# X1X1010/XequiNet

Measured on AMD Instinct MI355X. Metric: edges/sec + achieved HBM GB/s, energy+force inference, QM9-shape batch, higher is better.
Workload: dtype f32

## Files before the change

include/xeq.h:

```cpp
#ifndef XEQ_H
#define XEQ_H
#include <stdint.h>

#ifdef __cplusplus
extern "C" {
#endif

enum { XEQ_F32 = 0, XEQ_F64 = 1 };
enum { XEQ_RBF_BESSEL = 0, XEQ_RBF_GAUSSIAN = 1, XEQ_RBF_EXPBERN = 2, XEQ_RBF_EXPNORM = 3 };
enum { XEQ_CUTOFF_COSINE = 0, XEQ_CUTOFF_POLYNOMIAL = 1 };
enum {
  XEQ_OK = 0,
  XEQ_ERR_INVALID_ARGUMENT = 1,
  XEQ_ERR_LAUNCH = 2,
  XEQ_ERR_UNSUPPORTED = 3
};

int xeq_version(void);
const char* xeq_last_error(void);
int64_t xeq_launch_count(void);
int64_t xeq_launch_names(int64_t first, char* buf, int64_t cap);


int xeq_csr_rowptr(const int64_t* keys, int64_t n_keys, int64_t n_rows, int32_t* rowptr, void* stream);
// ... 236 lines not shown
int xeq_message_wq_supported(int num_basis, int node_dim, const int32_t mul[3]);
int xeq_message_wq_fits(int64_t n_nodes, int64_t n_edges, int num_basis, int node_dim, const int32_t mul[3]);
int64_t xeq_message_wq_pcap(int64_t n_nodes, int64_t n_edges);
int xeq_message_wq_waves(void);
int xeq_message_wq_record_floats_for(int num_basis);
int xeq_message_wq_record_floats(void);
int64_t xeq_message_wq_plan_workspace(int64_t n_nodes);
int64_t xeq_message_wq_win_ints(int n_ranges);
int xeq_message_wq_plan(const int32_t* rowptr, const int32_t* perm, const int64_t* owner, const int64_t* gather,
                        int64_t n_nodes, int64_t n_edges, int n_ranges, void* workspace, int64_t workspace_bytes,
                        int32_t* qptr, int32_t* pgath, int32_t* peid, int32_t* qinfo, int32_t* sq, int32_t* sn, int32_t* win,
                        void* stream);
int xeq_edge_basis_wq(const void* vec, int64_t n_nodes, int64_t n_edges, const int32_t* qptr, const int32_t* peid,
                      int rbf_kind, int cutoff_kind, int num_basis, double cutoff, const void* p0, const void* p1,
                      void* basis, void* dbasis, void* stream);
int xeq_message_fwd_wq(int64_t n_nodes, int64_t n_edges, int n_ranges, const int32_t* sq, const int32_t* sn, const int32_t* win,
                       const int32_t* c_rowptr, const int32_t* pgath, const int32_t* qinfo, const void* basis, const void* h,
                       const void* xhat, const void* s_in, const void* x_in, const void* w_rbf, const void* b_rbf,
                       int num_basis, int node_dim, const int32_t mul[3], void* s_out, void* x_out, int xhat_layout,
                       void* stream);
int64_t xeq_message_wq_parts_floats(int64_t n_nodes, int64_t n_edges, const int32_t mul[3]);
#define XEQ_XHAT_HIGHER_L_ZERO 2
#define XEQ_WQ_MIRROR_WALK 4
#define XEQ_WQ_PACKED_WEIGHTS 64
int64_t xeq_message_wq_packed_weight_floats(int num_basis, int node_dim, const int32_t mul[3]);
int xeq_message_wq_pack_weights(const void* w_rbf, const void* b_rbf, int num_basis, int node_dim, const int32_t mul[3], void* packed,
                                void* stream);
int xeq_message_bwd_wq(int64_t n_nodes, int64_t n_edges, int n_ranges, const int32_t* sq, const int32_t* sn, const int32_t* win,
                       const int32_t* n_rowptr, const int32_t* pgath, const int32_t* qinfo, const void* basis,
                       const void* dbasis, const void* h, const void* xhat, const void* grad_s, const void* grad_x,
                       const void* w_rbf, const void* b_rbf, int num_basis, int node_dim, const int32_t mul[3], void* grad_h,
                       void* grad_xhat, void* parts, int xhat_layout, void* stream);
int xeq_message_wq_table_max_rows(void);
int xeq_message_wq_first_table(int family, int64_t table_rows, int training, int per_node_front);
int xeq_edge_basis_wq_table(const void* vec, int64_t n_nodes, int64_t n_edges, const int32_t* qptr, const int32_t* peid,
                            int rbf_kind, int cutoff_kind, int num_basis, double cutoff, const void* p0, const void* p1,
                            void* basis, void* dbasis, const int32_t* pgath, const int32_t* qinfo, const void* z, int z_is_int64,
                            int64_t table_rows, int32_t* slot_rows, int32_t* quad_rows, void* stream);
int xeq_message_fwd_wq_table(int64_t n_nodes, int64_t n_edges, int n_ranges, const int32_t* sq, const int32_t* sn, const int32_t* win,
                             const int32_t* c_rowptr, const int32_t* slot_rows, const int32_t* qinfo, const void* basis,
                             const void* h_table, const void* xhat0_table, int64_t table_rows, const void* s_in, const void* x_in,
                             const void* w_rbf, const void* b_rbf, int num_basis, int node_dim, const int32_t mul[3], void* s_out,
                             void* x_out, int xhat_layout, void* stream);
int xeq_message_bwd_wq_table(int64_t n_nodes, int64_t n_edges, int n_ranges, const int32_t* sq, const int32_t* sn, const int32_t* win,
                             const int32_t* n_rowptr, const int32_t* pgath, const int32_t* qinfo, const int32_t* quad_rows,
                             const void* basis, const void* dbasis, const void* h_table, const void* xhat0_table, int64_t table_rows,
                             const void* grad_s, const void* grad_x, const void* w_rbf, const void* b_rbf, int num_basis, int node_dim,
                             const int32_t mul[3], void* parts, int xhat_layout, void* stream);
int xeq_message_wq_edge_grad(const void* vec, int64_t n_nodes, int64_t n_edges, const int32_t* qptr, const int32_t* peid,
                             const int32_t* mirror, const int32_t mul[3], const void* parts, void* grad_vec, void* stream);
#define XEQ_WQ_MAX_PART_SETS 8
int xeq_message_wq_edge_grad_sum(const void* vec, int64_t n_nodes, int64_t n_edges, const int32_t* qptr, const int32_t* peid,
                                 const int32_t* mirror, const int32_t mul[3], int n_sets, const void* const* parts, void* grad_vec,
                                 void* stream);


int xeq_norm_fwd(int dtype, const void* s, const void* x, const void* ln_w, const void* ln_b, const void* eq_w,
                 const void* eq_b, int64_t n, int node_dim, const int32_t mul[3], int do_norm, void* shat, int64_t ld_s,
                 void* xhat_bt, void* stats, void* stream);
int xeq_norm_bwd(int dtype, const void* s, const void* x, const void* ln_w, const void* eq_w, const void* stats,
                 int64_t n, int node_dim, const int32_t mul[3], int do_norm, const void* g_shat, int64_t ld_gs,
                 const void* g_xhat_bt, const void* res_s, const void* res_x, void* g_s, void* g_x, void* stream);
int xeq_uv_reduce_fwd(int dtype, const void* uv_bt, int64_t n, const int32_t mul[3], double eps, void* cat,
                      int64_t ld_cat, int node_dim, void* p, void* stream);
int xeq_uv_reduce_bwd(int dtype, const void* uv_bt, const void* g_p, const void* g_cat, int64_t ld_cat, int node_dim,
                      int64_t n, const int32_t mul[3], double eps, const void* g_x_out, const void* a, void* g_uv_bt,
// ... 145 lines not shown
```

xequinet_amd/csrc/xeq_message_wq.hip:

```cpp
#include "xeq_common.h"

#include <hipcub/hipcub.hpp>
#include <stdlib.h>

namespace xeq {

typedef float f32x16 __attribute__((ext_vector_type(16)));
typedef float f32x4 __attribute__((ext_vector_type(4)));
typedef int i32x4 __attribute__((ext_vector_type(4)));

typedef __bf16 bf16x8 __attribute__((ext_vector_type(8)));

constexpr bool wq_bftail(int ks) { return ks <= 3; }
constexpr int WQ_TAIL = 24;
constexpr int wq_tailw(int ks) { return ks <= 4 ? 4 : 8; }
constexpr int wq_recf(int ks) { return WQ_TAIL + 2 * wq_tailw(ks) + 8; }
constexpr int wq_yoff(int ks) { return WQ_TAIL + 2 * wq_tailw(ks); }
constexpr int wq_tail_values(int num_basis) { return (num_basis > 16 ? num_basis - 16 : 0) + 1; }
constexpr int wq_ks(int num_basis) {
  return wq_tail_values(num_basis) <= 1 ? 1 : (wq_tail_values(num_basis) <= 5 ? 3 : ((wq_tail_values(num_basis) + 1) / 2 < 4 ? 4 : (wq_tail_values(num_basis) + 1) / 2));
}
static_assert(wq_tailw(5) == wq_tailw(8) && wq_tailw(6) == wq_tailw(8) && wq_tailw(7) == wq_tailw(8) && !wq_bftail(5) && !wq_bftail(8),
              "records written for 5, 6 or 7 tail steps are read by the KS = 8 kernels");
constexpr int WQ_REC_MAX = 48;
// ... 343 lines not shown
  return 1;
}

__device__ __forceinline__ void wq_decode(const WqArgs& a, int nunits, int& s0, int& s1, int& unit) {
  const int b = blockIdx.x;
  int region, j;
  if (a.regions == 8) {
    region = b & 7;
    j = b >> 3;
  } else {
    region = 0;
    j = b;
  }
  const int c = j / nunits;
  unit = nunits - 1 - (j - c * nunits);
  const int base = region * a.region_steps, rend = min(base + a.region_steps, a.n_steps);
  s0 = s1 = 0;
  int cc = c;
#pragma unroll
  for (int v = 0; v < 3; ++v) {
    if (cc >= 0 && cc < a.lvl_chunks[v]) {
      const int lend = v < 2 ? base + a.lvl_start[v + 1] : rend;
      s0 = base + a.lvl_start[v] + cc * a.lvl_spw[v];
      s1 = min(s0 + a.lvl_spw[v], min(lend, rend));
    }
    cc -= a.lvl_chunks[v];
  }
}

#ifndef XEQ_WQ_WIN_FLOATS
#define XEQ_WQ_WIN_FLOATS 12288
#endif
constexpr int WQ_WIN_FLOATS = XEQ_WQ_WIN_FLOATS;
constexpr int WQ_TAB_MAX_ROWS = WQ_WIN_FLOATS * 4 / 512 < 128 ? WQ_WIN_FLOATS * 4 / 512 : 128;

template <int KS>
constexpr int WQ_WK = 3 * 64 * 4 + (wq_bftail(KS) ? 3 * 64 * 4 : KS * 64);
template <int KS>
__device__ __forceinline__ void wq_stage_weights(const WqArgs& a, const WqUnit& un, const float* __restrict__ w,
                                                 const float* __restrict__ b, float* wl) {
  const int nkind = un.l == 0 ? 3 : 2, B = a.B;
  if (a.packed_w) {
    const int unit_index = (un.l == 0 ? 0 : (un.l == 1 ? a.nu[0] : a.nu[0] + a.nu[1])) + un.cb;
    const f32x4* __restrict__ src = reinterpret_cast<const f32x4*>(w + (size_t)unit_index * (3 * WQ_WK<KS>));
    for (int idx = threadIdx.x; idx < nkind * WQ_WK<KS> / 4; idx += blockDim.x) reinterpret_cast<f32x4*>(wl)[idx] = src[idx];
    return;
  }
  auto row_of = [&](int kind, int ln) { return (kind == 0 ? un.u0 : (kind == 1 ? a.C + un.u0 : 2 * a.C + 32 * un.cb)) + (ln & 31); };
  for (int idx = threadIdx.x; idx < nkind * 3 * 64; idx += blockDim.x) {
    const int kind = idx / 192, rem = idx - 192 * kind, split = rem >> 6, ln = rem & 63;
    const int row = row_of(kind, ln), kh = ln >> 5;
    uint32_t pk[4] = {0u, 0u, 0u, 0u};
#pragma unroll
    for (int jj = 0; jj < 8; ++jj) {
      const int k = 8 * kh + jj;
      uint32_t a3[3];
      wq_split3(k < B ? w[(int64_t)row * B + k] : 0.f, a3[0], a3[1], a3[2]);
      pk[jj >> 1] |= a3[split] << (16 * (jj & 1));
    }
    *reinterpret_cast<f32x4*>(wl + kind * WQ_WK<KS> + 4 * (64 * split + ln)) =
        f32x4{__uint_as_float(pk[0]), __uint_as_float(pk[1]), __uint_as_float(pk[2]), __uint_as_float(pk[3])};
  }
  if constexpr (wq_bftail(KS)) {
    for (int idx = threadIdx.x; idx < nkind * 3 * 64; idx += blockDim.x) {
      const int kind = idx / 192, rem = idx - 192 * kind, v = rem >> 6, ln = rem & 63;
      const int row = row_of(kind, ln), kh = ln >> 5;
      uint32_t pk[4] = {0u, 0u, 0u, 0u};
#pragma unroll
      for (int jj = 0; jj < 8; ++jj) {
        const int slot = 8 * kh + jj, part = slot / 5, q = slot - 5 * part;
// ... 195 lines not shown
static __device__ unsigned long long g_wq_stamps[32];
static __device__ unsigned long long g_wq_wg[8192 * 4];
#ifdef XEQ_WQ_STAMPS
#define WQ_STAMP(i)                                                                                          \
  do {                                                                                                       \
    __builtin_amdgcn_sched_barrier(0);                                                                       \
    unsigned long long now_;                                                                                 \
    asm volatile("s_memtime %0\n\ts_waitcnt lgkmcnt(0)" : "=s"(now_)::"memory");                            \
    __builtin_amdgcn_sched_barrier(0);                                                                       \
    st_[i] += now_ - last_;                                                                                  \
    last_ = now_;                                                                                            \
  } while (0)
#else
#define WQ_STAMP(i) \
  do {              \
  } while (0)
#endif

__device__ __forceinline__ float wq_lds(const float* win, uint32_t byte_off) {
  return *reinterpret_cast<const float*>(reinterpret_cast<const char*>(win) + byte_off);
}
#ifndef XEQ_WQ_FWD_WPE
#define XEQ_WQ_FWD_WPE 2
#endif
#ifndef XEQ_WQ_BWD_WPE
#define XEQ_WQ_BWD_WPE 2
#endif

#ifndef XEQ_WQ_PART_BWD

template <int NM, bool XZ>
__device__ __forceinline__ void wq_stage_fwd(const WqArgs& a, const WqUnit& un, const WqCols& wc, const float* __restrict__ h,
                                             const float* __restrict__ xhat_, int w0, int nrows, float* win) {
  constexpr int NH = NM == 1 ? 3 : 2, NSL = NH + NM;
  if constexpr (XZ && NM > 1) {
    const int total = nrows * 8;
    for (int idx = threadIdx.x; idx < total; idx += blockDim.x) {
      const int row = idx >> 3, chunk = idx & 7;
      *reinterpret_cast<f32x4*>(win + (row * NSL + 1) * 32 + 4 * chunk) =
          *reinterpret_cast<const f32x4*>(h + (int64_t)(w0 + row) * a.H + a.C + un.u0 + 4 * chunk);
    }
    return;
  }
  const int total = nrows * NSL * 8;
  const int64_t xnode = wc.xnode_b / 4, xcomp = a.xl == 0 ? 32 : wc.xcomp_b / 4;
  constexpr int UN = 8;
  const int nthr = blockDim.x;
  for (int base = threadIdx.x; base < total; base += UN * nthr) {
    f32x4 v[UN];
#pragma unroll
    for (int k = 0; k < UN; ++k) {
      const int idx = base + k * nthr;
      const int piece = idx >> 3, chunk = idx & 7;
      const int row = piece / NSL, sl = piece - row * NSL;
      const int64_t n = w0 + (idx < total ? row : 0);
      const float* src = sl < NH ? h + n * a.H + (sl == 0 ? un.u0 : (sl == 1 ? a.C + un.u0 : 2 * a.C + 32 * un.cb))
                                 : xhat_ + wc.x_base + n * xnode + (sl - NH) * xcomp;
      v[k] = *reinterpret_cast<const f32x4*>(src + 4 * chunk);
    }
#pragma unroll
    for (int k = 0; k < UN; ++k) {
      const int idx = base + k * nthr;
      if (idx < total) *reinterpret_cast<f32x4*>(win + (idx >> 3) * 32 + 4 * (idx & 7)) = v[k];
    }
  }
}

constexpr int wq_tab_row_bytes(int NM) { return NM == 1 ? 512 : 128; }
template <int NM>
__device__ __forceinline__ void wq_stage_table_fwd(const WqArgs& a, const WqUnit& un, const float* __restrict__ h_tab,
                                                   const float* __restrict__ x0_tab, float* win) {
  constexpr int NP = NM == 1 ? 4 : 1;
  const int total = a.tab_rows * NP * 8;
  for (int idx = threadIdx.x; idx < total; idx += blockDim.x) {
    const int piece = idx >> 3, chunk = idx & 7;
    const int row = piece / NP, sl = piece - row * NP;
    const float* src = NM > 1 ? h_tab + (int64_t)row * a.H + a.C + un.u0
                              : (sl < 3 ? h_tab + (int64_t)row * a.H + (sl == 0 ? un.u0 : (sl == 1 ? a.C + un.u0 : 2 * a.C + 32 * un.cb))
                                        : x0_tab + (int64_t)row * a.F + un.u0);
    *reinterpret_cast<f32x4*>(win + piece * 32 + 4 * chunk) = *reinterpret_cast<const f32x4*>(src + 4 * chunk);
  }
}

template <int NM, int KS, bool WIN, bool XZ, bool FENCED, bool TAB = false>
__device__ __forceinline__ void wq_fwd_body(const WqArgs& a, int range, const WqUnit un, const WqCols& wc,
                                            const float* __restrict__ rec, const float* __restrict__ h,
                                            const float* __restrict__ xhat_, const float* __restrict__ s_in,
                                            const float* __restrict__ x_in, const float* wl, float* __restrict__ s_out,
                                            float* __restrict__ x_out, int* tbl, const float* win, int w0,
                                            unsigned long long* st_, unsigned long long& last_) {
  constexpr bool HAS_S = NM == 1;
  constexpr bool NO_STATE = XZ && NM > 1;
  constexpr int YOFF = NM == 3 ? 0 : 3;
  static_assert(!TAB || (WIN && (XZ || NM == 1)), "the table form is a window form of the first block");
  constexpr int NH = NM == 1 ? 3 : 2, ROWB = TAB ? wq_tab_row_bytes(NM) : (NH + NM) * 128;
  constexpr uint32_t HE_OFF = TAB && NM > 1 ? 0u : 128u;
  const int lane = threadIdx.x & 63, j = lane & 31, hh = lane >> 5;
  const uint32_t row_s = 4u * (uint32_t)a.F, row_x = 4u * (uint32_t)a.D;
  wq_for_isolated(a, range, lane, [&](int m) {
    if (hh == 0) {
      if constexpr (HAS_S) wq_st(s_out, (uint32_t)m * row_s + wc.b_s, wq_ld(s_in, (uint32_t)m * row_s + wc.b_s));
#pragma unroll
      for (int mm = 0; mm < NM; ++mm)
        wq_st(x_out, (uint32_t)m * row_x + wc.b_xe + 4u * mm, wq_ld(x_in, (uint32_t)m * row_x + wc.b_xe + 4u * mm));
    }
  });
  const WqStreams st = wq_streams(a, range, un.l == 0 ? a.mlong : 1);
  if (st.ntiles == 0) return;
  const float* __restrict__ h_e = h + a.C;
  const float* __restrict__ h_m = h + (2 * a.C + 32 * un.cb - un.u0);
  const float* xhat_m[NM];
#pragma unroll
  for (int m = 0; m < NM; ++m) xhat_m[m] = xhat_ + wc.x_base + (int64_t)m * (wc.xcomp_b / 4);
  const uint32_t stride0 = WIN ? (uint32_t)ROWB : 4u * (uint32_t)a.H, stride1 = WIN ? 0u : wc.xnode_b;
  const uint32_t gbase = WIN ? (uint32_t)w0 : 0u;
  uint32_t lxm[NM];
#pragma unroll
  for (int m = 0; m < NM; ++m) lxm[m] = (uint32_t)(NH * 128) + (a.xl == 0 ? 4u * (uint32_t)(j * NM + m) : (uint32_t)(128 * m + 4 * j));
  const float* Ws = wl;
  const float* We = wl + WQ_WK<KS>;
  const float* Wm = wl + 2 * WQ_WK<KS>;

  float acc_s = 0.f, acc_x[NM];
#pragma unroll
  for (int m = 0; m < NM; ++m) acc_x[m] = 0.f;

  using Row = WqRow<KS, 1, (NM > 1)>;
  Row row;
  wq_row<KS, 1, (NM > 1)>(a, st, lane, 0, rec, nullptr, row, (int)gbase);
  wq_publish<KS, 1, (NM > 1)>(lane, row, stride0, stride1, tbl, gbase);
  __builtin_amdgcn_wave_barrier();

#ifdef XEQ_WQ_DEFER_STORES
  constexpr bool DEFER_ST = NM <= 3;
#else
  constexpr bool DEFER_ST = false;
#endif
  float pend_x[DEFER_ST ? 4 : 1][NM], pend_s[DEFER_ST ? 4 : 1];
  uint32_t pend_ob[DEFER_ST ? 4 : 1], pend_os[DEFER_ST ? 4 : 1];
  int pend_last[DEFER_ST ? 4 : 1];
  if constexpr (DEFER_ST) {
#pragma unroll
    for (int g = 0; g < 4; ++g) pend_last[g] = 0;
  }
  auto flush_nodes = [&]() {
    if constexpr (DEFER_ST) {
#pragma unroll
      for (int g = 0; g < 4; ++g)
        if (pend_last[g]) {
#pragma unroll
          for (int m = 0; m < NM; ++m) wq_st(x_out, pend_ob[g] + 4u * m, pend_x[g][m]);
// ... 14 lines not shown
#pragma unroll
    for (int g = 0; g < 4; ++g) {
      uint32_t t0[4];
      wq_tread4<uint32_t>(tb, T_G0 + 16 * hh + 4 * g, t0);
#pragma unroll
      for (int r = 0; r < 4; ++r) g0[4 * g + r] = t0[r];
      if constexpr (!WIN) {
        uint32_t t1[4];
        wq_tread4<uint32_t>(tb, T_G1 + 16 * hh + 4 * g, t1);
#pragma unroll
        for (int r = 0; r < 4; ++r) g1[4 * g + r] = t1[r];
      }
      const uint32_t own = (uint32_t)tb[T_QOWN + 4 * hh + g];
      keep[g] = tb[T_QKEEP + 4 * hh + g];
      last[g] = tb[T_QLAST + 4 * hh + g];
      ob[g] = own * row_x + wc.b_xe;
      os[g] = own * row_s + wc.b_s;
#pragma unroll
      for (int m = 0; m < NM; ++m) res_x[g][m] = wq_ld(x_in, ob[g] + 4u * m);
      res_s[g] = HAS_S ? wq_ld(s_in, os[g]) : 0.f;
    }
    XEQ_WQ_FSB();
    wq_row<KS, 1, (NM > 1)>(a, st, lane, t + 1, rec, nullptr, row, (int)gbase);
    XEQ_WQ_FSB();
    WQ_STAMP(5);
#ifdef XEQ_WQ_FWD_GR
    constexpr int GR = NM == 5 && XEQ_WQ_FWD_GR > 4 ? XEQ_WQ_FWD_GR / 2 : XEQ_WQ_FWD_GR;
#else
    constexpr int GR = NM == 5 ? 8 : 16;
#endif
    f32x16 ds, de, dm;
#pragma unroll
    for (int r0 = 0; r0 < 16; r0 += GR) {
      float hs[GR], he[GR], hm[HAS_S ? GR : 1], xv[GR][NM];
#pragma unroll
      for (int u = 0; u < GR; ++u) {
        const int v = r0 + u;
        if constexpr (WIN) {
          const uint32_t oh = g0[v] + 4u * (uint32_t)j;
          if constexpr (!NO_STATE) hs[u] = wq_lds(win, oh);
          he[u] = wq_lds(win, oh + HE_OFF);
          if constexpr (HAS_S) hm[u] = wq_lds(win, oh + 256u);
          if constexpr (!NO_STATE) {
#pragma unroll
            for (int m = 0; m < NM; ++m) xv[u][m] = wq_lds(win, g0[v] + lxm[m]);
          }
        } else {
          const uint32_t oh = g0[v] + wc.b_hs, ox = g1[v] + wc.b_x;
          if constexpr (!NO_STATE) hs[u] = wq_ld(h, oh);
          he[u] = wq_ld(h_e, oh);
          if constexpr (HAS_S) hm[u] = wq_ld(h_m, oh);
          if constexpr (!NO_STATE) {
#pragma unroll
            for (int m = 0; m < NM; ++m) xv[u][m] = wq_ld(xhat_m[m], ox);
          }
        }
      }
      XEQ_WQ_FSB();
      WQ_STAMP(6);
      if (r0 == 0) {
        de = wq_filter<KS>(R, We, lane);
        ds = de;
        if constexpr (!NO_STATE) ds = wq_filter<KS>(R, Ws, lane);
        dm = ds;
        if constexpr (HAS_S) dm = wq_filter<KS>(R, Wm, lane);
        XEQ_WQ_FSB();
        WQ_STAMP(7);
      }
#pragma unroll
      for (int g = r0 / 4; g < (r0 + GR) / 4; ++g) {
        float Y[NM][4];
        if constexpr (NM > 1) {
#pragma unroll
          for (int m = 0; m < NM; ++m) wq_tread4<float>(tb, T_Y + 32 * (YOFF + m) + 16 * hh + 4 * g, Y[m]);
        }
        float xq[NM], sq = 0.f;
#pragma unroll
        for (int m = 0; m < NM; ++m) xq[m] = 0.f;
#pragma unroll
        for (int r = 0; r < 4; ++r) {
          const int v = 4 * g + r, u = v - r0;
          const float ge = he[u] * de[v];
          if constexpr (NO_STATE) {
#pragma unroll
            for (int m = 0; m < NM; ++m) xq[m] = __builtin_fmaf(Y[m][r], ge, xq[m]);
          } else {
            const float gs = hs[u] * ds[v];
#pragma unroll
            for (int m = 0; m < NM; ++m) xq[m] = __builtin_fmaf(xv[u][m], gs, NM > 1 ? __builtin_fmaf(Y[m][r], ge, xq[m]) : xq[m] + ge);
          }
          if constexpr (HAS_S) sq = __builtin_fmaf(hm[u], dm[v], sq);
        }
#pragma unroll
        for (int m = 0; m < NM; ++m) acc_x[m] = (keep[g] ? acc_x[m] : res_x[g][m]) + xq[m];
        if constexpr (HAS_S) acc_s = (keep[g] ? acc_s : res_s[g]) + sq;
        if constexpr (DEFER_ST) {
#pragma unroll
          for (int m = 0; m < NM; ++m) pend_x[g][m] = acc_x[m];
          pend_s[g] = acc_s;
          pend_ob[g] = ob[g];
          pend_os[g] = os[g];
          pend_last[g] = last[g];
        } else if (last[g]) {
#pragma unroll
          for (int m = 0; m < NM; ++m) wq_st(x_out, ob[g] + 4u * m, acc_x[m]);
          if constexpr (HAS_S) wq_st(s_out, os[g], acc_s);
        }
      }
      if constexpr (GR < 16) XEQ_WQ_FSB();
      WQ_STAMP(8);
    }
    wq_publish<KS, 1, (NM > 1)>(lane, row, stride0, stride1, tnext, gbase);
    __builtin_amdgcn_wave_barrier();
    WQ_STAMP(9);
  }
  flush_nodes();
}


template <int NM, int KS, bool XZ, bool FENCED, bool TAB = false>
__device__ __forceinline__ void wq_fwd_role(const WqArgs& a, int s_beg, int s_end, const WqUnit un, const float* __restrict__ rec,
                                            const float* __restrict__ h, const float* __restrict__ xhat,
                                            const float* __restrict__ s_in, const float* __restrict__ x_in, const float* wl,
                                            float* __restrict__ s_out, float* __restrict__ x_out, int* tbl, float* win) {
  constexpr int NH = NM == 1 ? 3 : 2, ROWB = (NH + NM) * 128;
  const WqCols wc = wq_cols<NM>(a, un, threadIdx.x & 31);
  unsigned long long st_[16] = {0, 0, 0, 0, 0, 0, 0, 0, 0, 0, 0, 0, 0, 0, 0, 0}, last_ = 0;
#ifdef XEQ_WQ_STAMPS
  last_ = __builtin_amdgcn_s_memtime();
#endif
  const WqClass cl = wq_class(a, un.l);
  const int c_beg = cl.m == a.mlong ? s_beg : s_beg * a.mlong, c_end = min(cl.m == a.mlong ? s_end : s_end * a.mlong, cl.n_steps);
  if constexpr (TAB) {
    for (int step = c_beg; step < c_end; ++step) {
      const int range = step * WQ_WAVES + __builtin_amdgcn_readfirstlane((int)(threadIdx.x >> 6));
      if (range < cl.n_ranges) wq_fwd_body<NM, KS, true, XZ, FENCED, true>(a, range, un, wc, rec, h, xhat, s_in, x_in, wl, s_out, x_out, tbl, win, 0, st_, last_);
    }
    return;
  }
  for (int step = c_beg; step < c_end; ++step) {
    const int w0 = cl.win[2 * step], nrows = cl.win[2 * step + 1];
#ifdef XEQ_WQ_NO_WINDOW
    const bool use_win = false;
#else
    const bool use_win = nrows > 0 && nrows * ROWB <= WQ_WIN_FLOATS * 4;
#endif
    WQ_STAMP(0);
    if (use_win) wq_stage_fwd<NM, XZ>(a, un, wc, h, xhat, w0, nrows, win);
    WQ_STAMP(1);
    __syncthreads();
    WQ_STAMP(2);
    const int range = step * WQ_WAVES + __builtin_amdgcn_readfirstlane((int)(threadIdx.x >> 6));
    if (range < cl.n_ranges) {
      if (use_win) wq_fwd_body<NM, KS, true, XZ, FENCED>(a, range, un, wc, rec, h, xhat, s_in, x_in, wl, s_out, x_out, tbl, win, w0, st_, last_);
      else wq_fwd_body<NM, KS, false, XZ, FENCED>(a, range, un, wc, rec, h, xhat, s_in, x_in, wl, s_out, x_out, tbl, win, 0, st_, last_);
    }
    WQ_STAMP(3);
    __syncthreads();
    WQ_STAMP(10);
  }
#ifdef XEQ_WQ_STAMPS
  if (NM == 1 && (threadIdx.x & 63) == 0) {
    for (int i = 0; i < 11; ++i) atomicAdd(&g_wq_stamps[i], st_[i]);
    atomicAdd(&g_wq_stamps[15], 1ull);
  }
#endif
}

template <int KS>
__global__ void __launch_bounds__(256) k_wq_pack_weights(WqArgs a, const float* __restrict__ w, const float* __restrict__ b, float* __restrict__ out) {
  const WqUnit un = wq_unit(a, (int)blockIdx.x);
  float* dst = out + (size_t)blockIdx.x * (3 * WQ_WK<KS>);
  if (un.l != 0)
    for (int idx = threadIdx.x; idx < WQ_WK<KS>; idx += blockDim.x) dst[2 * WQ_WK<KS> + idx] = 0.f;
  wq_stage_weights<KS>(a, un, w, b, dst);
}

template <int KS, bool XZ, bool TAB = false>
__global__ void __launch_bounds__(64 * WQ_WAVES) __attribute__((amdgpu_waves_per_eu(XEQ_WQ_FWD_WPE)))
k_message_fwd_wq(WqArgs a, const float* __restrict__ rec, const float* __restrict__ h, const float* __restrict__ xhat,
                 const float* __restrict__ s_in, const float* __restrict__ x_in, const float* __restrict__ w_rbf,
                 const float* __restrict__ b_rbf, float* __restrict__ s_out, float* __restrict__ x_out) {
  __shared__ __attribute__((aligned(16))) float win[WQ_WIN_FLOATS];
  __shared__ __attribute__((aligned(16))) int tbl_all[WQ_WAVES][2 * T_SIZE];
  __shared__ __attribute__((aligned(16))) float wl[3 * WQ_WK<KS>];
  int s_beg, s_end, unit;
  wq_decode(a, a.nu[0] + a.nu[1] + a.nu[2], s_beg, s_end, unit);
  if (s_beg >= s_end) return;
  const WqUnit un = wq_unit(a, unit);
  wq_stage_weights<KS>(a, un, w_rbf, b_rbf, wl);
  if constexpr (TAB) {
    static_assert(XZ, "the table form is a first-block form");
    if (un.l == 0) wq_stage_table_fwd<1>(a, un, h, xhat, win);
    else wq_stage_table_fwd<3>(a, un, h, xhat, win);
  }
  __syncthreads();
  int* tbl = tbl_all[threadIdx.x >> 6];
#ifdef XEQ_WQ_ONLY_L
  if (un.l == XEQ_WQ_ONLY_L) wq_fwd_role<2 * XEQ_WQ_ONLY_L + 1, KS, XZ, !XZ>(a, s_beg, s_end, un, rec, h, xhat, s_in, x_in, wl, s_out, x_out, tbl, win);
  return;
#endif
#ifdef XEQ_WQ_ROLE_TIME_FWD
  unsigned long long rr0_;
  asm volatile("s_memrealtime %0\n\ts_waitcnt lgkmcnt(0)" : "=s"(rr0_)::"memory");
#endif
  if (un.l == 0) wq_fwd_role<1, KS, false, !XZ, TAB>(a, s_beg, s_end, un, rec, h, xhat, s_in, x_in, wl, s_out, x_out, tbl, win);
  else if (un.l == 1) wq_fwd_role<3, KS, XZ, !XZ, TAB>(a, s_beg, s_end, un, rec, h, xhat, s_in, x_in, wl, s_out, x_out, tbl, win);
  else wq_fwd_role<5, KS, XZ, !XZ, TAB>(a, s_beg, s_end, un, rec, h, xhat, s_in, x_in, wl, s_out, x_out, tbl, win);
#ifdef XEQ_WQ_ROLE_TIME_FWD
  if (threadIdx.x == 0 && blockIdx.x < 8192) {
    unsigned long long rr1_;
    unsigned hw, xcc;
    asm volatile("s_waitcnt vmcnt(0)\n\ts_memrealtime %0\n\ts_getreg_b32 %1, hwreg(HW_REG_HW_ID)\n\ts_getreg_b32 %2, hwreg(HW_REG_XCC_ID)\n\ts_waitcnt lgkmcnt(0)"
                 : "=s"(rr1_), "=s"(hw), "=s"(xcc)::"memory");
    g_wq_wg[4 * blockIdx.x + 0] = hw | ((unsigned long long)un.l << 32);
    g_wq_wg[4 * blockIdx.x + 1] = xcc;
    g_wq_wg[4 * blockIdx.x + 2] = rr0_;
    g_wq_wg[4 * blockIdx.x + 3] = rr1_;
  }
#endif
}

#endif
#ifdef XEQ_WQ_PART_BWD
struct WqParts {
  float* pd;
  float* y1;
  float* y2;
  int64_t P;
};

#define XEQ_WQ_DPP(v, ctrl) __builtin_bit_cast(float, __builtin_amdgcn_update_dpp(0, __builtin_bit_cast(int, (v)), ctrl, 0xF, 0xF, true))
__device__ __forceinline__ float wq_red_ab(float r0, float r1, float r2, float r3, bool b0, bool b1) {
  const float a0 = (b0 ? r2 : r0) + XEQ_WQ_DPP(b0 ? r0 : r2, 0xB1);
  const float a1 = (b0 ? r3 : r1) + XEQ_WQ_DPP(b0 ? r1 : r3, 0xB1);
  return (b1 ? a1 : a0) + XEQ_WQ_DPP(b1 ? a0 : a1, 0x4E);
}
__device__ __forceinline__ float wq_xor4(float v) {
  const float t = XEQ_WQ_DPP(v, 0x1B);
  return XEQ_WQ_DPP(t, 0x141);
}
// ... 647 lines not shown
  do {                                                                                                                       \
    const int ks = wq_ks(num_basis);                                                                                         \
    if (ks <= 1) hipLaunchKernelGGL((KERNEL<1, FLAG>), grid, dim3(64 * WQ_WAVES), 0, (hipStream_t)stream, __VA_ARGS__);      \
    else if (ks <= 3) hipLaunchKernelGGL((KERNEL<3, FLAG>), grid, dim3(64 * WQ_WAVES), 0, (hipStream_t)stream, __VA_ARGS__); \
    else if (ks <= 4) hipLaunchKernelGGL((KERNEL<4, FLAG>), grid, dim3(64 * WQ_WAVES), 0, (hipStream_t)stream, __VA_ARGS__); \
    else hipLaunchKernelGGL((KERNEL<8, FLAG>), grid, dim3(64 * WQ_WAVES), 0, (hipStream_t)stream, __VA_ARGS__);              \
  } while (0)
#define XEQ_WQ_DISPATCH(KERNEL, flag, ...)                   \
  do {                                                       \
    if (flag) XEQ_WQ_DISPATCH_KS(KERNEL, true, __VA_ARGS__); \
    else XEQ_WQ_DISPATCH_KS(KERNEL, false, __VA_ARGS__);     \
  } while (0)

#define XEQ_WQ_DISPATCH_TAB(KERNEL, ...)                                                                                    \
  do {                                                                                                                      \
    const int ks = wq_ks(num_basis);                                                                                        \
    if (ks <= 1) hipLaunchKernelGGL((KERNEL<1, true, true>), grid, dim3(64 * WQ_WAVES), 0, (hipStream_t)stream, __VA_ARGS__);      \
    else if (ks <= 3) hipLaunchKernelGGL((KERNEL<3, true, true>), grid, dim3(64 * WQ_WAVES), 0, (hipStream_t)stream, __VA_ARGS__); \
    else if (ks <= 4) hipLaunchKernelGGL((KERNEL<4, true, true>), grid, dim3(64 * WQ_WAVES), 0, (hipStream_t)stream, __VA_ARGS__); \
    else hipLaunchKernelGGL((KERNEL<8, true, true>), grid, dim3(64 * WQ_WAVES), 0, (hipStream_t)stream, __VA_ARGS__);              \
  } while (0)
#define XEQ_WQ_CHECK_TABLE(who, rows, tab, hint)                                                                                  \
  do {                                                                                                                            \
    XEQ_CHECK_ARG((rows) >= 1 && (rows) <= WQ_TAB_MAX_ROWS, who ": the element table has %lld rows, the table form takes 1 .. %d", \
                  (long long)(rows), WQ_TAB_MAX_ROWS);                                                                            \
    XEQ_CHECK_ARG((tab) != nullptr && h_table != nullptr && xhat0_table != nullptr, who ": NULL table argument");                 \
    XEQ_CHECK_ARG(((hint) & 1) && ((hint) & XEQ_XHAT_HIGHER_L_ZERO), who ": the table form is the first block's (BT layout, XEQ_XHAT_HIGHER_L_ZERO)"); \
  } while (0)

extern "C" {

#ifndef XEQ_WQ_PART_BWD
int xeq_message_wq_table_max_rows(void) { return WQ_TAB_MAX_ROWS; }

int xeq_message_wq_supported(int num_basis, int node_dim, const int32_t mul[3]) { return wq_supported(num_basis, node_dim, mul) ? 1 : 0; }

int xeq_message_wq_fits(int64_t n_nodes, int64_t n_edges, int num_basis, int node_dim, const int32_t mul[3]) {
  return wq_supported(num_basis, node_dim, mul) && n_nodes < (1ll << 30) && wq_fits(n_nodes, n_edges, node_dim, mul) ? 1 : 0;
}

int64_t xeq_message_wq_pcap(int64_t n_nodes, int64_t n_edges) { return wq_pcap(n_nodes, n_edges); }

int xeq_message_wq_waves(void) { return WQ_WAVES; }

int xeq_message_wq_record_floats(void) { return wq_recf(4); }
int xeq_message_wq_record_floats_for(int num_basis) { return wq_recf(wq_ks(num_basis)); }

int64_t xeq_message_wq_plan_workspace(int64_t n_nodes) {
  size_t temp = 0;
  QuadCount op{nullptr, n_nodes};
  hipcub::CountingInputIterator<int64_t> cnt(0);
  hipcub::TransformInputIterator<int32_t, QuadCount, hipcub::CountingInputIterator<int64_t>> it(cnt, op);
  if (hipcub::DeviceScan::ExclusiveSum(nullptr, temp, it, (int32_t*)nullptr, (int)(n_nodes + 1)) != hipSuccess) return -1;
  return (int64_t)temp + 256;
}

int xeq_message_wq_plan(const int32_t* rowptr, const int32_t* perm, const int64_t* owner, const int64_t* gather,
                        int64_t n_nodes, int64_t n_edges, int n_ranges, void* workspace, int64_t workspace_bytes,
                        int32_t* qptr, int32_t* pgath, int32_t* peid, int32_t* qinfo, int32_t* sq, int32_t* sn, int32_t* win,
                        void* stream) {
  XEQ_CHECK_ARG(n_nodes >= 0 && n_edges >= 0 && n_ranges >= 1 && n_nodes < (1ll << 30) && n_edges < (1ll << 31), "xeq_message_wq_plan: bad sizes");
  const int64_t need = xeq_message_wq_plan_workspace(n_nodes);
  XEQ_CHECK_ARG(need >= 0 && workspace_bytes >= need, "xeq_message_wq_plan: workspace of %lld bytes, need %lld", (long long)workspace_bytes, (long long)need);
  QuadCount op{rowptr, n_nodes};
  if (n_nodes <= SCAN_WG_MAX_ITEMS) {
    static const bool attr_ok = hipFuncSetAttribute((const void*)k_wq_quad_scan, hipFuncAttributeMaxDynamicSharedMemorySize,
// ... 271 lines not shown
```

xequinet_amd/lib.py:

```python
from __future__ import annotations

import ctypes
import os
from ctypes import c_char_p, c_double, c_int, c_int32, c_int64, c_uint64, c_void_p
from typing import Optional

import torch

_HERE = os.path.dirname(os.path.abspath(__file__))
LIB_PATH = os.environ.get("XEQ_LIB_PATH") or os.path.join(_HERE, "libxeq_hip.so")

XEQ_F32, XEQ_F64 = 0, 1
COPY_MANY_MAX = 16
MD_CHUNK = 256
FIRE_FRESH, FIRE_ACTIVE, FIRE_CONVERGED = 0, 1, 2
SB_ACCUM_VEC = 16
XHAT_HIGHER_L_ZERO = 2
SB_Y0_ZERO = 8
SB_Q_ACCUMULATE = 16
SB_NO_GY = 32
WQ_MIRROR_WALK = 4
WQ_PACKED_WEIGHTS = 64
WQ_MAX_PART_SETS = 8
RBF_KINDS = {"bessel": 0, "gaussian": 1, "expbern": 2, "expnorm": 3}
# ... 87 lines not shown
    "xeq_norm_param_grad": [_P, _P, _P, _P, c_int64, _P, c_int64, c_int, _I3, c_int, _P, _P],
    "xeq_message_auto_family": [c_int, c_int64, c_int64, c_int, c_int, _I3],
    "xeq_message_wq_edges_per_stream": [c_int64, c_int64],
    "xeq_edge_basis_width": [c_int],
    "xeq_edge_basis": [c_int, _P, c_int64, c_int, c_int, c_int, c_double, _P, _P, _P, _P, _P],
    "xeq_message_fwd_sb": [c_int, c_int64, c_int64, _P, _P, _P, _P, _P, _P, _P, _P, _P, _P, c_int, c_int, _I3, _P, _P, c_int, _P],
    "xeq_message_bwd_sbq": [c_int, c_int64, c_int64, _P, _P, _P, _P, _P, _P, _P, _P, _P, _P, c_int, c_int, _I3, _P, _P, _P, _P, c_int, _P],
    "xeq_message_q_wgrad": [c_int, _P, _P, c_int64, c_int, c_int, _I3, c_int, _P, _P],
    "xeq_message_q_wgrad_chunks": [c_int64],
    "xeq_train_norm": [c_int, c_int, c_int64, _P, _P, _P, _P, _P, _P, _P, _P, _P, _P, c_int, _I3, c_double, c_double, c_int, _P, _P, _P, _P],
    "xeq_train_uv": [c_int, c_int, c_int64, _P, _P, _P, _I3, c_double, _P, _P, _P],
    "xeq_train_out": [c_int, c_int, c_int64, _P, _P, _P, _P, _P, _P, _P, _P, c_int, _I3, _P, _P, _P, _P],
    "xeq_train_edge_supported": [c_int, c_int, c_int, c_int],
    "xeq_train_edge": [c_int, c_int, c_int64, _P, _P, _P, _P, c_int, c_int, c_int, c_double, _P, _P, _P, _P],
    "xeq_zero_rows_from": [_P, c_int64, c_int64, _P, _P],
    "xeq_message_fwd_sb_pair": [c_int, c_int64, c_int64, _P, _P, _P, _P, _P, _P, _P, _P, _P, _P, _P, _P, _P, c_int, c_int, _I3, _P, _P, c_int, _P],
    "xeq_message_bwd_sbq_pair": [c_int, c_int64, c_int64, _P, _P, _P, _P, _P, _P, _P, _P, _P, _P, _P, _P, _P, c_int, c_int, _I3, _P, _P, _P, _P, c_int, _P],
    "xeq_message_bwd_sb": [c_int, c_int64, c_int64, _P, _P, _P, _P, _P, _P, _P, _P, _P, _P, _P, c_int, c_int, _I3, _P, _P, _P,
                           c_int, _P],
    "xeq_message_sb_fits": [c_int64, c_int64, c_int, c_int, _I3],
    "xeq_message_wq_supported": [c_int, c_int, _I3],
    "xeq_message_wq_fits": [c_int64, c_int64, c_int, c_int, _I3],
    "xeq_message_wq_pcap": [c_int64, c_int64],
    "xeq_message_wq_waves": [],
    "xeq_message_wq_record_floats": [],
    "xeq_message_wq_record_floats_for": [c_int],
    "xeq_message_wq_plan_workspace": [c_int64],
    "xeq_message_wq_win_ints": [c_int],
    "xeq_message_wq_plan": [_P, _P, _P, _P, c_int64, c_int64, c_int, _P, c_int64, _P, _P, _P, _P, _P, _P, _P, _P],
    "xeq_edge_basis_wq": [_P, c_int64, c_int64, _P, _P, c_int, c_int, c_int, c_double, _P, _P, _P, _P, _P],
    "xeq_message_fwd_wq": [c_int64, c_int64, c_int, _P, _P, _P, _P, _P, _P, _P, _P, _P, _P, _P, _P, _P, c_int, c_int, _I3,
                           _P, _P, c_int, _P],
    "xeq_message_wq_table_max_rows": [],
    "xeq_message_wq_first_table": [c_int, c_int64, c_int, c_int],
    "xeq_edge_basis_wq_table": [_P, c_int64, c_int64, _P, _P, c_int, c_int, c_int, c_double, _P, _P, _P, _P, _P, _P, _P, c_int, c_int64, _P, _P, _P],
    "xeq_message_fwd_wq_table": [c_int64, c_int64, c_int, _P, _P, _P, _P, _P, _P, _P, _P, _P, c_int64, _P, _P, _P, _P, c_int, c_int, _I3,
                                 _P, _P, c_int, _P],
    "xeq_message_bwd_wq_table": [c_int64, c_int64, c_int, _P, _P, _P, _P, _P, _P, _P, _P, _P, _P, _P, c_int64, _P, _P, _P, _P, c_int, c_int,
                                 _I3, _P, c_int, _P],
    "xeq_message_wq_parts_floats": [c_int64, c_int64, _I3],
    "xeq_message_bwd_wq": [c_int64, c_int64, c_int, _P, _P, _P, _P, _P, _P, _P, _P, _P, _P, _P, _P, _P, _P, c_int, c_int,
                           _I3, _P, _P, _P, c_int, _P],
    "xeq_message_wq_packed_weight_floats": [c_int, c_int, _I3],
    "xeq_message_wq_pack_weights": [_P, _P, c_int, c_int, _I3, _P, _P],
    "xeq_message_wq_edge_grad": [_P, c_int64, c_int64, _P, _P, _P, _I3, _P, _P, _P],
    "xeq_message_wq_edge_grad_sum": [_P, c_int64, c_int64, _P, _P, _P, _I3, c_int, ctypes.POINTER(c_void_p), _P, _P],
    "xeq_norm_fwd": [c_int, _P, _P, _P, _P, _P, _P, c_int64, c_int, _I3, c_int, _P, c_int64, _P, _P, _P],
    "xeq_norm_bwd": [c_int, _P, _P, _P, _P, _P, c_int64, c_int, _I3, c_int, _P, c_int64, _P, _P, _P, _P, _P, _P],
    "xeq_uv_reduce_fwd": [c_int, _P, c_int64, _I3, c_double, _P, c_int64, c_int, _P, _P],
    "xeq_uv_reduce_bwd": [c_int, _P, _P, _P, c_int64, c_int, c_int64, _I3, c_double, _P, _P, _P, _P],
    "xeq_update_out_fwd": [c_int, _P, _P, _P, _P, _P, c_int64, c_int, _I3, _P, _P, _P],
    "xeq_update_out_bwd": [c_int, _P, _P, _P, _P, _P, c_int64, c_int, _I3, _P, _P, _P, _P],
    "xeq_update_uv_supported": [c_int, c_int, _I3],
    "xeq_update_uv_fwd": [_P, _P, _P, _P, _P, _P, c_int64, c_int, _I3, c_int, _P, _P, _P, c_int, c_double, _P, c_int64, _P, _P, _P, _P],
    "xeq_update_uv_bwd": [_P, _P, _P, c_int64, _P, _P, _P, c_int64, _P, _P, _P, _P, _P, c_int64, c_int, _I3, c_int, _P, _P, _P, c_double,
                          _P, _P, _P, _P],
    "xeq_mlp2_supported": [c_int, c_int, c_int, c_int],
    "xeq_node_tile_split": [c_int64, c_int, ctypes.POINTER(c_int64)],
    "xeq_mlp_packed_floats": [c_int, c_int],
    "xeq_mlp_pack": [_P, _P, c_int, c_int, c_int, _P, _P],
    "xeq_mlp2_fwd": [_P, c_int64, c_int64, c_int, _P, _P, c_int, _P, _P, c_int64, _P],
    "xeq_mlp2_bwd": [_P, c_int64, c_int64, c_int, _P, _P, _P, c_int, _P, c_int64, _P],
    "xeq_mlp2h_supported": [c_int, c_int, c_int, c_int],
    "xeq_mlp2h_fwd": [c_int, _P, c_int64, c_int64, c_int, c_int, _P, _P, c_int, _P, _P, c_int64, _P],
    "xeq_mlp2h_bwd": [c_int, _P, c_int64, c_int64, c_int, c_int, _P, _P, _P, c_int, _P, c_int64, _P],
    "xeq_mlp2_and_linear": [c_int, _P, c_int64, c_int64, c_int, _P, _P, c_int, _P, _P, c_int64, _P, c_int64, c_int, _P, c_int, _P, c_int64, _P],
# ... 162 lines not shown
```

Before: 186.1 million.

## Pre-multiply gate into staged window rows and extend l>0 window into unused weight block

```diff
diff --git a/include/xeq.h b/include/xeq.h
--- a/include/xeq.h
+++ b/include/xeq.h
@@ -292,6 +292,8 @@
                        const void* w_rbf, const void* b_rbf, int num_basis, int node_dim, const int32_t mul[3], void* grad_h,
                        void* grad_xhat, void* parts, int xhat_layout, void* stream);
 int xeq_message_wq_table_max_rows(void);
+int xeq_message_wq_window_bytes(int l);
+int xeq_message_wq_window_rows(int l, int first_block);
 int xeq_message_wq_first_table(int family, int64_t table_rows, int training, int per_node_front);
 int xeq_edge_basis_wq_table(const void* vec, int64_t n_nodes, int64_t n_edges, const int32_t* qptr, const int32_t* peid,
                             int rbf_kind, int cutoff_kind, int num_basis, double cutoff, const void* p0, const void* p1,
diff --git a/profiles/wq_window_overflow.py b/profiles/wq_window_overflow.py
--- /dev/null
+++ b/profiles/wq_window_overflow.py
@@ -0,0 +1,36 @@
+import os
+import sys
+
+import numpy as np
+import torch
+
+ROOT = os.path.dirname(os.path.dirname(os.path.abspath(__file__)))
+sys.path.insert(0, ROOT)
+from xequinet_amd import lib, ops
+from xequinet_amd.data import NeighborTransform, XequiBatch
+from xequinet_amd.data import synthetic as syn
+from xequinet_amd.nn import resolve_model
+
+
+def main(workload="qm9_1024"):
+    L = lib.load()
+    pos, z, ptr, _ = syn.make_workload(workload)
+    rc = resolve_model("xpainn").cutoff_radius
+    t = lambda a, dt=None: torch.tensor(a, dtype=dt).to("cuda")
+    batch = NeighborTransform(rc)(XequiBatch(t(pos, torch.float32), t(z), t(ptr)))
+    n, ei = len(pos), batch.edge_index
+    graph = ops.EdgeGraph(ei, n)
+    eps = ops._wq_edges_per_stream(graph.n_edges, n)
+    plan = graph.wq_plan(False, eps)
+    steps = -(-plan["n_ranges"] // int(L.xeq_message_wq_waves()))
+    rows = plan["win"].cpu().numpy().reshape(-1, 2)[:steps, 1]
+    print(f"{workload}: N = {n}, E = {graph.n_edges}, {eps} edges per stream, {plan['n_ranges']} ranges, {steps} steps")
+    print(f"window rows per step: min {rows.min()}, median {int(np.median(rows))}, mean {rows.mean():.1f}, max {rows.max()}")
+    base = 48 * 1024
+    for l, (old, new) in enumerate(((512, 384), (640, 512), (896, 768))):
+        caps = (("older rows", base // old), ("product rows, 48 KB", base // new), ("this build", int(L.xeq_message_wq_window_rows(l, 0))))
+        print(f"l = {l}: " + "; ".join(f"{name}: {cap} rows, {100.0 * float((rows <= cap).mean()):.1f} % of steps fit" for name, cap in caps))
+
+
+if __name__ == "__main__":
+    main(*sys.argv[1:2])
diff --git a/xequinet_amd/csrc/xeq_message_wq.hip b/xequinet_amd/csrc/xeq_message_wq.hip
--- a/xequinet_amd/csrc/xeq_message_wq.hip
+++ b/xequinet_amd/csrc/xeq_message_wq.hip
@@ -399,10 +399,19 @@
 #define XEQ_WQ_WIN_FLOATS 12288
 #endif
 constexpr int WQ_WIN_FLOATS = XEQ_WQ_WIN_FLOATS;
-constexpr int WQ_TAB_MAX_ROWS = WQ_WIN_FLOATS * 4 / 512 < 128 ? WQ_WIN_FLOATS * 4 / 512 : 128;
+constexpr int wq_fwd_row_bytes(int nm, bool xz, bool tab) { return nm > 1 && tab ? 128 : (nm > 1 && xz ? (2 + nm) * 128 : (nm + (nm == 1 ? 2 : 1)) * 128); }
+constexpr uint32_t wq_fwd_he_off(int nm, bool xz, bool tab) { return nm > 1 && tab ? 0u : (nm > 1 && xz ? 128u : 128u * (uint32_t)nm); }
+#ifndef XEQ_WQ_WIN_EXT
+#define XEQ_WQ_WIN_EXT 1024
+#endif
+constexpr int WQ_WIN_EXT = XEQ_WQ_WIN_EXT;
+constexpr int wq_fwd_win_floats(int l) { return WQ_WIN_FLOATS + (l > 0 ? WQ_WIN_EXT : 0); }
+constexpr int WQ_TAB_MAX_ROWS = WQ_WIN_FLOATS * 4 / wq_fwd_row_bytes(1, true, true) < 128 ? WQ_WIN_FLOATS * 4 / wq_fwd_row_bytes(1, true, true) : 128;
 
 template <int KS>
 constexpr int WQ_WK = 3 * 64 * 4 + (wq_bftail(KS) ? 3 * 64 * 4 : KS * 64);
+static_assert(WQ_WK<1> >= WQ_WIN_EXT && WQ_WK<3> >= WQ_WIN_EXT && WQ_WK<4> >= WQ_WIN_EXT && WQ_WK<8> >= WQ_WIN_EXT && WQ_WIN_EXT % 4 == 0,
+              "the window extension of the l > 0 units lies inside their unused third weight block");
 template <int KS>
 __device__ __forceinline__ void wq_stage_weights(const WqArgs& a, const WqUnit& un, const float* __restrict__ w,
                                                  const float* __restrict__ b, float* wl) {
@@ -664,8 +673,8 @@
 template <int NM, bool XZ>
 __device__ __forceinline__ void wq_stage_fwd(const WqArgs& a, const WqUnit& un, const WqCols& wc, const float* __restrict__ h,
                                              const float* __restrict__ xhat_, int w0, int nrows, float* win) {
-  constexpr int NH = NM == 1 ? 3 : 2, NSL = NH + NM;
   if constexpr (XZ && NM > 1) {
+    constexpr int NSL = wq_fwd_row_bytes(NM, true, false) / 128;
     const int total = nrows * 8;
     for (int idx = threadIdx.x; idx < total; idx += blockDim.x) {
       const int row = idx >> 3, chunk = idx & 7;
@@ -673,44 +682,70 @@
           *reinterpret_cast<const f32x4*>(h + (int64_t)(w0 + row) * a.H + a.C + un.u0 + 4 * chunk);
     }
     return;
-  }
-  const int total = nrows * NSL * 8;
-  const int64_t xnode = wc.xnode_b / 4, xcomp = a.xl == 0 ? 32 : wc.xcomp_b / 4;
-  constexpr int UN = 8;
-  const int nthr = blockDim.x;
-  for (int base = threadIdx.x; base < total; base += UN * nthr) {
-    f32x4 v[UN];
-#pragma unroll
-    for (int k = 0; k < UN; ++k) {
-      const int idx = base + k * nthr;
-      const int piece = idx >> 3, chunk = idx & 7;
-      const int row = piece / NSL, sl = piece - row * NSL;
-      const int64_t n = w0 + (idx < total ? row : 0);
-      const float* src = sl < NH ? h + n * a.H + (sl == 0 ? un.u0 : (sl == 1 ? a.C + un.u0 : 2 * a.C + 32 * un.cb))
-                                 : xhat_ + wc.x_base + n * xnode + (sl - NH) * xcomp;
-      v[k] = *reinterpret_cast<const f32x4*>(src + 4 * chunk);
-    }
-#pragma unroll
-    for (int k = 0; k < UN; ++k) {
-      const int idx = base + k * nthr;
-      if (idx < total) *reinterpret_cast<f32x4*>(win + (idx >> 3) * 32 + 4 * (idx & 7)) = v[k];
-    }
-  }
-}
-
-constexpr int wq_tab_row_bytes(int NM) { return NM == 1 ? 512 : 128; }
+  } else {
+    constexpr int NSL = wq_fwd_row_bytes(NM, false, false) / 128;
+    constexpr int UN = NM == 1 ? 2 : 1;
+    const int total = nrows * 8;
+    const int64_t xnode = wc.xnode_b / 4, xcomp = wc.xcomp_b / 4;
+    const bool e3 = a.xl == 0;
+    const int nthr = blockDim.x;
+    for (int base = threadIdx.x; base < total; base += UN * nthr) {
+      f32x4 gs[UN], ge[UN], gm[UN], x[UN][NM];
+#pragma unroll
+      for (int k = 0; k < UN; ++k) {
+        const int idx = base + k * nthr, chunk = idx & 7;
+        const int64_t n = w0 + (idx < total ? idx >> 3 : 0);
+        const float* hrow = h + n * a.H + 4 * chunk;
+        gs[k] = *reinterpret_cast<const f32x4*>(hrow + un.u0);
+        ge[k] = *reinterpret_cast<const f32x4*>(hrow + a.C + un.u0);
+        if constexpr (NM == 1) gm[k] = *reinterpret_cast<const f32x4*>(hrow + 2 * a.C + 32 * un.cb);
+        const float* xrow = xhat_ + wc.x_base + n * xnode;
+#pragma unroll
+        for (int q = 0; q < NM; ++q)
+          x[k][q] = *reinterpret_cast<const f32x4*>(xrow + (e3 ? 4 * chunk * NM + 4 * q : q * xcomp + 4 * chunk));
+      }
+#pragma unroll
+      for (int k = 0; k < UN; ++k) {
+        const int idx = base + k * nthr, chunk = idx & 7;
+        if (idx < total) {
+          float* dst = win + (idx >> 3) * (NSL * 32);
+#pragma unroll
+          for (int q = 0; q < NM; ++q) {
+            f32x4 p;
+#pragma unroll
+            for (int i = 0; i < 4; ++i) p[i] = (e3 ? gs[k][(4 * q + i) / NM] : gs[k][i]) * x[k][q][i];
+            *reinterpret_cast<f32x4*>(dst + (e3 ? 4 * chunk * NM + 4 * q : 32 * q + 4 * chunk)) = p;
+          }
+          *reinterpret_cast<f32x4*>(dst + 32 * NM + 4 * chunk) = ge[k];
+          if constexpr (NM == 1) *reinterpret_cast<f32x4*>(dst + 32 * NM + 32 + 4 * chunk) = gm[k];
+        }
+      }
+    }
+  }
+}
+
 template <int NM>
 __device__ __forceinline__ void wq_stage_table_fwd(const WqArgs& a, const WqUnit& un, const float* __restrict__ h_tab,
                                                    const float* __restrict__ x0_tab, float* win) {
-  constexpr int NP = NM == 1 ? 4 : 1;
-  const int total = a.tab_rows * NP * 8;
+  constexpr int NP = wq_fwd_row_bytes(NM, true, true) / 128;
+  const int total = a.tab_rows * 8;
   for (int idx = threadIdx.x; idx < total; idx += blockDim.x) {
-    const int piece = idx >> 3, chunk = idx & 7;
-    const int row = piece / NP, sl = piece - row * NP;
-    const float* src = NM > 1 ? h_tab + (int64_t)row * a.H + a.C + un.u0
-                              : (sl < 3 ? h_tab + (int64_t)row * a.H + (sl == 0 ? un.u0 : (sl == 1 ? a.C + un.u0 : 2 * a.C + 32 * un.cb))
-                                        : x0_tab + (int64_t)row * a.F + un.u0);
-    *reinterpret_cast<f32x4*>(win + piece * 32 + 4 * chunk) = *reinterpret_cast<const f32x4*>(src + 4 * chunk);
+    const int row = idx >> 3, chunk = idx & 7;
+    const float* hrow = h_tab + (int64_t)row * a.H + 4 * chunk;
+    float* dst = win + row * (NP * 32) + 4 * chunk;
+    if constexpr (NM > 1) {
+      *reinterpret_cast<f32x4*>(dst) = *reinterpret_cast<const f32x4*>(hrow + a.C + un.u0);
+    } else {
+      const f32x4 gs = *reinterpret_cast<const f32x4*>(hrow + un.u0), ge = *reinterpret_cast<const f32x4*>(hrow + a.C + un.u0);
+      const f32x4 gm = *reinterpret_cast<const f32x4*>(hrow + 2 * a.C + 32 * un.cb);
+      const f32x4 x0 = *reinterpret_cast<const f32x4*>(x0_tab + (int64_t)row * a.F + un.u0 + 4 * chunk);
+      f32x4 p;
+#pragma unroll
+      for (int i = 0; i < 4; ++i) p[i] = gs[i] * x0[i];
+      *reinterpret_cast<f32x4*>(dst) = p;
+      *reinterpret_cast<f32x4*>(dst + 32) = ge;
+      *reinterpret_cast<f32x4*>(dst + 64) = gm;
+    }
   }
 }
 
@@ -725,8 +760,8 @@
   constexpr bool NO_STATE = XZ && NM > 1;
   constexpr int YOFF = NM == 3 ? 0 : 3;
   static_assert(!TAB || (WIN && (XZ || NM == 1)), "the table form is a window form of the first block");
-  constexpr int NH = NM == 1 ? 3 : 2, ROWB = TAB ? wq_tab_row_bytes(NM) : (NH + NM) * 128;
-  constexpr uint32_t HE_OFF = TAB && NM > 1 ? 0u : 128u;
+  constexpr int ROWB = wq_fwd_row_bytes(NM, XZ, TAB);
+  constexpr uint32_t HE_OFF = wq_fwd_he_off(NM, XZ, TAB);
   const int lane = threadIdx.x & 63, j = lane & 31, hh = lane >> 5;
   const uint32_t row_s = 4u * (uint32_t)a.F, row_x = 4u * (uint32_t)a.D;
   wq_for_isolated(a, range, lane, [&](int m) {
@@ -748,7 +783,7 @@
   const uint32_t gbase = WIN ? (uint32_t)w0 : 0u;
   uint32_t lxm[NM];
 #pragma unroll
-  for (int m = 0; m < NM; ++m) lxm[m] = (uint32_t)(NH * 128) + (a.xl == 0 ? 4u * (uint32_t)(j * NM + m) : (uint32_t)(128 * m + 4 * j));
+  for (int m = 0; m < NM; ++m) lxm[m] = a.xl == 0 ? 4u * (uint32_t)(j * NM + m) : (uint32_t)(128 * m + 4 * j);
   const float* Ws = wl;
   const float* We = wl + WQ_WK<KS>;
   const float* Wm = wl + 2 * WQ_WK<KS>;
@@ -829,15 +864,14 @@
     f32x16 ds, de, dm;
 #pragma unroll
     for (int r0 = 0; r0 < 16; r0 += GR) {
-      float hs[GR], he[GR], hm[HAS_S ? GR : 1], xv[GR][NM];
+      float hs[WIN ? 1 : GR], he[GR], hm[HAS_S ? GR : 1], xv[GR][NM];
 #pragma unroll
       for (int u = 0; u < GR; ++u) {
         const int v = r0 + u;
         if constexpr (WIN) {
           const uint32_t oh = g0[v] + 4u * (uint32_t)j;
-          if constexpr (!NO_STATE) hs[u] = wq_lds(win, oh);
           he[u] = wq_lds(win, oh + HE_OFF);
-          if constexpr (HAS_S) hm[u] = wq_lds(win, oh + 256u);
+          if constexpr (HAS_S) hm[u] = wq_lds(win, oh + HE_OFF + 128u);
           if constexpr (!NO_STATE) {
 #pragma unroll
             for (int m = 0; m < NM; ++m) xv[u][m] = wq_lds(win, g0[v] + lxm[m]);
@@ -882,9 +916,12 @@
 #pragma unroll
             for (int m = 0; m < NM; ++m) xq[m] = __builtin_fmaf(Y[m][r], ge, xq[m]);
           } else {
-            const float gs = hs[u] * ds[v];
-#pragma unroll
-            for (int m = 0; m < NM; ++m) xq[m] = __builtin_fmaf(xv[u][m], gs, NM > 1 ? __builtin_fmaf(Y[m][r], ge, xq[m]) : xq[m] + ge);
+#pragma unroll
+            for (int m = 0; m < NM; ++m) {
+              float pm = xv[u][m];
+              if constexpr (!WIN) pm = hs[u] * xv[u][m];
+              xq[m] = __builtin_fmaf(ds[v], pm, NM > 1 ? __builtin_fmaf(Y[m][r], ge, xq[m]) : xq[m] + ge);
+            }
           }
           if constexpr (HAS_S) sq = __builtin_fmaf(hm[u], dm[v], sq);
         }
@@ -920,7 +957,7 @@
                                             const float* __restrict__ h, const float* __restrict__ xhat,
                                             const float* __restrict__ s_in, const float* __restrict__ x_in, const float* wl,
                                             float* __restrict__ s_out, float* __restrict__ x_out, int* tbl, float* win) {
-  constexpr int NH = NM == 1 ? 3 : 2, ROWB = (NH + NM) * 128;
+  constexpr int ROWB = wq_fwd_row_bytes(NM, XZ, false), WIN_BYTES = wq_fwd_win_floats(NM > 1 ? 1 : 0) * 4;
   const WqCols wc = wq_cols<NM>(a, un, threadIdx.x & 31);
   unsigned long long st_[16] = {0, 0, 0, 0, 0, 0, 0, 0, 0, 0, 0, 0, 0, 0, 0, 0}, last_ = 0;
 #ifdef XEQ_WQ_STAMPS
@@ -940,7 +977,7 @@
 #ifdef XEQ_WQ_NO_WINDOW
     const bool use_win = false;
 #else
-    const bool use_win = nrows > 0 && nrows * ROWB <= WQ_WIN_FLOATS * 4;
+    const bool use_win = nrows > 0 && nrows <= WIN_BYTES / ROWB;
 #endif
     WQ_STAMP(0);
     if (use_win) wq_stage_fwd<NM, XZ>(a, un, wc, h, xhat, w0, nrows, win);
@@ -978,9 +1015,11 @@
 k_message_fwd_wq(WqArgs a, const float* __restrict__ rec, const float* __restrict__ h, const float* __restrict__ xhat,
                  const float* __restrict__ s_in, const float* __restrict__ x_in, const float* __restrict__ w_rbf,
                  const float* __restrict__ b_rbf, float* __restrict__ s_out, float* __restrict__ x_out) {
-  __shared__ __attribute__((aligned(16))) float win[WQ_WIN_FLOATS];
+  __shared__ __attribute__((aligned(16))) float lds[3 * WQ_WK<KS> + WQ_WIN_FLOATS];
   __shared__ __attribute__((aligned(16))) int tbl_all[WQ_WAVES][2 * T_SIZE];
-  __shared__ __attribute__((aligned(16))) float wl[3 * WQ_WK<KS>];
+  float* const wl = lds;
+  float* const win0 = lds + 3 * WQ_WK<KS>;
+  float* const win12 = win0 - WQ_WIN_EXT;
   int s_beg, s_end, unit;
   wq_decode(a, a.nu[0] + a.nu[1] + a.nu[2], s_beg, s_end, unit);
   if (s_beg >= s_end) return;
@@ -988,22 +1027,22 @@
   wq_stage_weights<KS>(a, un, w_rbf, b_rbf, wl);
   if constexpr (TAB) {
     static_assert(XZ, "the table form is a first-block form");
-    if (un.l == 0) wq_stage_table_fwd<1>(a, un, h, xhat, win);
-    else wq_stage_table_fwd<3>(a, un, h, xhat, win);
+    if (un.l == 0) wq_stage_table_fwd<1>(a, un, h, xhat, win0);
+    else wq_stage_table_fwd<3>(a, un, h, xhat, win12);
   }
   __syncthreads();
   int* tbl = tbl_all[threadIdx.x >> 6];
 #ifdef XEQ_WQ_ONLY_L
-  if (un.l == XEQ_WQ_ONLY_L) wq_fwd_role<2 * XEQ_WQ_ONLY_L + 1, KS, XZ, !XZ>(a, s_beg, s_end, un, rec, h, xhat, s_in, x_in, wl, s_out, x_out, tbl, win);
+  if (un.l == XEQ_WQ_ONLY_L) wq_fwd_role<2 * XEQ_WQ_ONLY_L + 1, KS, XZ, !XZ>(a, s_beg, s_end, un, rec, h, xhat, s_in, x_in, wl, s_out, x_out, tbl, XEQ_WQ_ONLY_L ? win12 : win0);
   return;
 #endif
 #ifdef XEQ_WQ_ROLE_TIME_FWD
   unsigned long long rr0_;
   asm volatile("s_memrealtime %0\n\ts_waitcnt lgkmcnt(0)" : "=s"(rr0_)::"memory");
 #endif
-  if (un.l == 0) wq_fwd_role<1, KS, false, !XZ, TAB>(a, s_beg, s_end, un, rec, h, xhat, s_in, x_in, wl, s_out, x_out, tbl, win);
-  else if (un.l == 1) wq_fwd_role<3, KS, XZ, !XZ, TAB>(a, s_beg, s_end, un, rec, h, xhat, s_in, x_in, wl, s_out, x_out, tbl, win);
-  else wq_fwd_role<5, KS, XZ, !XZ, TAB>(a, s_beg, s_end, un, rec, h, xhat, s_in, x_in, wl, s_out, x_out, tbl, win);
+  if (un.l == 0) wq_fwd_role<1, KS, false, !XZ, TAB>(a, s_beg, s_end, un, rec, h, xhat, s_in, x_in, wl, s_out, x_out, tbl, win0);
+  else if (un.l == 1) wq_fwd_role<3, KS, XZ, !XZ, TAB>(a, s_beg, s_end, un, rec, h, xhat, s_in, x_in, wl, s_out, x_out, tbl, win12);
+  else wq_fwd_role<5, KS, XZ, !XZ, TAB>(a, s_beg, s_end, un, rec, h, xhat, s_in, x_in, wl, s_out, x_out, tbl, win12);
 #ifdef XEQ_WQ_ROLE_TIME_FWD
   if (threadIdx.x == 0 && blockIdx.x < 8192) {
     unsigned long long rr1_;
@@ -1717,6 +1756,12 @@
 
 #ifndef XEQ_WQ_PART_BWD
 int xeq_message_wq_table_max_rows(void) { return WQ_TAB_MAX_ROWS; }
+
+int xeq_message_wq_window_bytes(int l) { return l < 0 || l > 2 ? -1 : wq_fwd_win_floats(l) * 4; }
+int xeq_message_wq_window_rows(int l, int first_block) {
+  if (l < 0 || l > 2) return -1;
+  return wq_fwd_win_floats(l) * 4 / wq_fwd_row_bytes(2 * l + 1, first_block != 0, false);
+}
 
 int xeq_message_wq_supported(int num_basis, int node_dim, const int32_t mul[3]) { return wq_supported(num_basis, node_dim, mul) ? 1 : 0; }
 
diff --git a/xequinet_amd/lib.py b/xequinet_amd/lib.py
--- a/xequinet_amd/lib.py
+++ b/xequinet_amd/lib.py
@@ -143,6 +143,8 @@
     "xeq_message_fwd_wq": [c_int64, c_int64, c_int, _P, _P, _P, _P, _P, _P, _P, _P, _P, _P, _P, _P, _P, c_int, c_int, _I3,
                            _P, _P, c_int, _P],
     "xeq_message_wq_table_max_rows": [],
+    "xeq_message_wq_window_bytes": [c_int],
+    "xeq_message_wq_window_rows": [c_int, c_int],
     "xeq_message_wq_first_table": [c_int, c_int64, c_int, c_int],
     "xeq_edge_basis_wq_table": [_P, c_int64, c_int64, _P, _P, c_int, c_int, c_int, c_double, _P, _P, _P, _P, _P, _P, _P, c_int, c_int64, _P, _P, _P],
     "xeq_message_fwd_wq_table": [c_int64, c_int64, c_int, _P, _P, _P, _P, _P, _P, _P, _P, _P, c_int64, _P, _P, _P, _P, c_int, c_int, _I3,
```

Result: slower. 183.8 million (-1.2%).
